# hediet/slideo

Hardware: AMD Instinct MI355X
Metric: frames/sec matched (1080p vs 500-page ORB set) (higher is better)
Workload: dtype u8

## Files before the change

### slideo_amd/csrc/orb.hip.h

```cpp
#pragma once
#include <limits.h>
#include <hip/hip_runtime.h>
#include <stdint.h>

#include "geom.h"
#include "types.h"
#include "cv_math.hip.h"

namespace slideo {

__global__ __launch_bounds__(256) void gray_kernel(const uint8_t* __restrict__ frames, int64_t frame_stride,
                                                   int stride, uint8_t* __restrict__ pyr, int64_t pyr_frame_bytes,
                                                   int w, int h, int pitch, int aligned4, GrayCoef gc) {
    const uint32_t half = 1u << (gc.shift - 1);
    auto gray_of = [&](uint32_t b, uint32_t g, uint32_t r) { return (__umul24(b, gc.cb) + __umul24(g, gc.cg) + __umul24(r, gc.cr) + half) >> gc.shift; };
    const int x = (blockIdx.x * 256 + threadIdx.x) * 4;
    const int y = blockIdx.y;
    if (x >= w) return;
    const uint8_t* src = frames + (int64_t)blockIdx.z * frame_stride + (int64_t)y * stride + (int64_t)x * 3;
    uint8_t* dst = pyr + (int64_t)blockIdx.z * pyr_frame_bytes + (int64_t)y * pitch + x;
    if (aligned4 && x + 3 < w) {
        const uint32_t* s = reinterpret_cast<const uint32_t*>(src);
        uint32_t a = s[0], b = s[1], c = s[2];
        uint32_t g0 = gray_of(a & 255, (a >> 8) & 255, (a >> 16) & 255);
        uint32_t g1 = gray_of(a >> 24, b & 255, (b >> 8) & 255);
        uint32_t g2 = gray_of((b >> 16) & 255, b >> 24, c & 255);
        uint32_t g3 = gray_of((c >> 8) & 255, (c >> 16) & 255, c >> 24);
        *reinterpret_cast<uint32_t*>(dst) = g0 | (g1 << 8) | (g2 << 16) | (g3 << 24);
    } else {
        for (int i = 0; i < 4 && x + i < w; ++i)
            dst[i] = (uint8_t)gray_of(src[3 * i], src[3 * i + 1], src[3 * i + 2]);
    }
}

__device__ __forceinline__ uint32_t dot2_u16(uint32_t a, uint32_t b, uint32_t c = 0u) {
    typedef unsigned short u16x2 __attribute__((ext_vector_type(2)));
    return __builtin_amdgcn_udot2(__builtin_bit_cast(u16x2, a), __builtin_bit_cast(u16x2, b), c, false);
}

constexpr int RESIZE_ROWS = 4;

__global__ __launch_bounds__(256) void resize_kernel(uint8_t* __restrict__ pyr, int64_t pyr_frame_bytes,
                                                     LevelGeom src, LevelGeom dst,
                                                     const uint32_t* __restrict__ lin_tab, int nxq, uint32_t nxq_magic) {
    const uint32_t t = blockIdx.x * 256 + threadIdx.x;
    const int yg = nxq_magic ? (int)__umulhi(t, nxq_magic) : (int)t;
    const int y0 = yg * RESIZE_ROWS;
    if (y0 >= dst.h) return;
    const int x0 = ((int)t - (int)__umul24(yg, nxq)) * 4;
    uint8_t* base = pyr + (int64_t)blockIdx.z * pyr_frame_bytes;
    const int nx = min(4, dst.w - x0);
    const uint4 xq = *reinterpret_cast<const uint4*>(lin_tab + dst.xtab_ofs + x0);
    const uint4 cq = *reinterpret_cast<const uint4*>(lin_tab + dst.xctab_ofs + x0);
    uint32_t ye[RESIZE_ROWS];
#pragma unroll
    for (int r = 0; r < RESIZE_ROWS; ++r) ye[r] = lin_tab[dst.ytab_ofs + min(y0 + r, dst.h - 1)];
    const uint32_t xe[4] = {xq.x, xq.y, xq.z, xq.w};
    const uint32_t cp[4] = {cq.x, cq.y, cq.z, cq.w};
    const int xs = min((int)(xe[0] & 0xffff), src.pitch - 8);
    const bool narrow = (int)(xe[3] & 0xffff) + 1 - xs < 8 || ((int)(xe[3] & 0xffff) - xs < 8 && (xe[3] >> 16) == 0);
    uint2 a[RESIZE_ROWS], b[RESIZE_ROWS];
#pragma unroll
    for (int r = 0; r < RESIZE_ROWS; ++r) {
        const int yo = ye[r] & 0xffff;
        const uint8_t* p0 = base + src.ofs + __umul24(yo, src.pitch) + xs;
        const uint8_t* p1 = base + src.ofs + __umul24(min(yo + 1, src.h - 1), src.pitch) + xs;
        __builtin_memcpy(&a[r], p0, 8);
        __builtin_memcpy(&b[r], p1, 8);
    }
#pragma unroll
    for (int r = 0; r < RESIZE_ROWS; ++r) {
        const int y = y0 + r;
        if (y >= dst.h) break;
        const int yo = ye[r] & 0xffff, cy1 = ye[r] >> 16, cy0 = 256 - cy1;
        uint32_t v[4];
        if (narrow) {
#pragma unroll
            for (int i = 0; i < 4; ++i) {
                const uint32_t pq = (uint32_t)((int)(xe[i] & 0xffff) - xs);
                const uint32_t sel = pq * 0x00010001u + 0x0c010c00u;
                const uint32_t ta = __builtin_amdgcn_perm(a[r].y, a[r].x, sel);
                const uint32_t tb = __builtin_amdgcn_perm(b[r].y, b[r].x, sel);
                v[i] = __umul24(cy0, dot2_u16(ta, cp[i])) + (__umul24(cy1, dot2_u16(tb, cp[i])) + (1u << 15));
            }
        } else {
            const uint8_t* r0 = base + src.ofs + __umul24(yo, src.pitch);
            const uint8_t* r1 = base + src.ofs + __umul24(min(yo + 1, src.h - 1), src.pitch);
#pragma unroll
            for (int i = 0; i < 4; ++i) {
                const int xo = xe[i] & 0xffff, cx1 = xe[i] >> 16, cx0 = 256 - cx1;
                const int xo1 = min(xo + 1, src.w - 1);
                uint32_t h0 = (uint32_t)cx0 * r0[xo] + (uint32_t)cx1 * r0[xo1];
                uint32_t h1 = (uint32_t)cx0 * r1[xo] + (uint32_t)cx1 * r1[xo1];
                v[i] = (uint32_t)cy0 * h0 + (uint32_t)cy1 * h1 + (1u << 15);
            }
        }
        const uint32_t outv = __builtin_amdgcn_perm(__builtin_amdgcn_perm(v[3], v[2], 0x0c0c0602u),
                                                    __builtin_amdgcn_perm(v[1], v[0], 0x0c0c0602u), 0x05040100u);
        uint8_t* d = base + dst.ofs + __umul24(y, dst.pitch) + x0;
        if (nx == 4) *reinterpret_cast<uint32_t*>(d) = outv;
        else for (int i = 0; i < nx; ++i) d[i] = (uint8_t)(outv >> (8 * i));
    }
}

__global__ __launch_bounds__(256) void resize_quad_kernel(uint8_t* __restrict__ pyr, int64_t pyr_frame_bytes,
                                                          LevelGeom src, LevelGeom dst,
                                                          const uint32_t* __restrict__ lin_tab, int nxq, uint32_t nxq_magic) {
    const uint32_t t = blockIdx.x * 256 + threadIdx.x;
    const uint32_t yg = nxq_magic ? __umulhi(t, nxq_magic) : t;
    const uint32_t y0 = yg * 4u;
    if ((int)y0 >= dst.h) return;
    const uint32_t q = t - __umul24(yg, (uint32_t)nxq);
    const uint8_t* __restrict__ sbase = pyr + (int64_t)blockIdx.z * pyr_frame_bytes + src.ofs;
    uint8_t* __restrict__ dbase = pyr + (int64_t)blockIdx.z * pyr_frame_bytes + dst.ofs;
    const uint4 sel4 = reinterpret_cast<const uint4*>(lin_tab + dst.xsel_ofs)[q];
    const uint4 cp4 = reinterpret_cast<const uint4*>(lin_tab + dst.xctab_ofs)[q];
    const uint32_t xs = lin_tab[dst.xs_ofs + q];
    const uint4 ye4 = *reinterpret_cast<const uint4*>(lin_tab + dst.ytab_ofs + y0);
    const uint32_t ye[4] = {ye4.x, ye4.y, ye4.z, ye4.w};
    const uint32_t sel[4] = {sel4.x, sel4.y, sel4.z, sel4.w}, cp[4] = {cp4.x, cp4.y, cp4.z, cp4.w};
    uint2 a[4], b[4];
#pragma unroll
    for (int r = 0; r < 4; ++r) {
        const uint32_t yo = ye[r] & 0xffffu;
        const uint32_t o0 = __umul24(yo, (uint32_t)src.pitch) + xs;
        const uint32_t o1 = __umul24(min(yo + 1u, (uint32_t)(src.h - 1)), (uint32_t)src.pitch) + xs;
        {
            const uint32_t sh = (xs & 3u) * 8u;
            uint32_t w0[3], w1[3];
            __builtin_memcpy(w0, sbase + (o0 & ~3u), 12);
            __builtin_memcpy(w1, sbase + (o1 & ~3u), 12);
            a[r] = make_uint2(__builtin_amdgcn_alignbit(w0[1], w0[0], sh), __builtin_amdgcn_alignbit(w0[2], w0[1], sh));
            b[r] = make_uint2(__builtin_amdgcn_alignbit(w1[1], w1[0], sh), __builtin_amdgcn_alignbit(w1[2], w1[1], sh));
        }
    }
    const uint32_t dofs = __umul24(y0, (uint32_t)dst.pitch) + 4u * q;
#pragma unroll
    for (int r = 0; r < 4; ++r) {
        const uint32_t cy1 = ye[r] >> 16, cy0 = 256u - cy1;
        uint32_t v[4];
#pragma unroll
        for (int i = 0; i < 4; ++i) {
            const uint32_t ta = __builtin_amdgcn_perm(a[r].y, a[r].x, sel[i]);
            const uint32_t tb = __builtin_amdgcn_perm(b[r].y, b[r].x, sel[i]);
            v[i] = __umul24(cy0, dot2_u16(ta, cp[i])) + (__umul24(cy1, dot2_u16(tb, cp[i])) + (1u << 15));
        }
        const uint32_t outv = __builtin_amdgcn_perm(__builtin_amdgcn_perm(v[3], v[2], 0x0c0c0602u),
                                                    __builtin_amdgcn_perm(v[1], v[0], 0x0c0c0602u), 0x05040100u);
        if ((int)(y0 + r) < dst.h) *reinterpret_cast<uint32_t*>(dbase + (dofs + (uint32_t)r * (uint32_t)dst.pitch)) = outv;
    }
}

__device__ __forceinline__ bool run9(uint32_t m) {
    m |= m << 16;
    m &= m >> 1; m &= m >> 2; m &= m >> 4; m &= m >> 1;
    return m != 0;
}

__device__ __forceinline__ int level_of_tile(const PyrGeom& g, int tile, bool blur) {
    int l = 0;
    for (int i = 1; i < g.nlevels; ++i) {
        int t0 = blur ? g.lv[i].btile0 : g.lv[i].ftile0;
        int n = blur ? g.lv[i].btx * g.lv[i].bty : g.lv[i].ftx * g.lv[i].fty;
        if (n > 0 && tile >= t0) l = i;
    }
    return l;
}

constexpr int FAST_SW = FAST_TW + 2, FAST_SH = FAST_TH + 2;
constexpr int FAST_XO = 4;
constexpr int FAST_RW = FAST_TW + 14, FAST_RH = FAST_TH + 8;
static_assert(FAST_SW == 128 && FAST_RW % 4 == 0 && (FAST_RW / 4) % 2 == 1 && FAST_RW >= FAST_SW + FAST_XO + 3, "fast_kernel maps one score row onto two wave-widths");

typedef short fast_s2 __attribute__((ext_vector_type(2)));
typedef unsigned short fast_us2 __attribute__((ext_vector_type(2)));
__device__ __forceinline__ fast_s2 fast_swap(fast_s2 a) { return __builtin_shufflevector(a, a, 1, 0); }

#ifndef FAST_TPB_V
#define FAST_TPB_V 8
#endif
constexpr int FAST_TPB = FAST_TPB_V;
constexpr int FAST_STAGE_CAP = 128;
constexpr int FAST_NDW = FAST_RW / 4;
constexpr int FAST_NLD = (FAST_RH + 6) / 7;

struct FastTile { int l, x0, y0; };

inline int4 fast_tile_entry(const PyrGeom& g, int tile_id) {
    int l = 0;
    for (int i = 1; i < g.nlevels; ++i) if (g.lv[i].ftx * g.lv[i].fty > 0 && tile_id >= g.lv[i].ftile0) l = i;
    const LevelGeom& L = g.lv[l];
    const int tile = tile_id - L.ftile0, ty = tile / (L.ftx > 0 ? L.ftx : 1), tx = tile - ty * L.ftx;
    const int x0 = L.rx0 + tx * FAST_TW, y0 = L.ry0 + ty * FAST_TH;
    return make_int4(l, x0, y0, 0);
}

__device__ __forceinline__ FastTile fast_tile_geo(const int4* __restrict__ tab, int tile_id) {
    const int4 e = tab[tile_id];
    FastTile T;
    T.l = e.x; T.x0 = e.y; T.y0 = e.z;
    return T;
}

__device__ __forceinline__ FastTile fast_tile_geo(const PyrGeom& g, int tile_id) {
    FastTile T;
    T.l = level_of_tile(g, tile_id, false);
    const LevelGeom& L = g.lv[T.l];
    const int tile = tile_id - L.ftile0;
    const int ty = tile / L.ftx, tx = tile - ty * L.ftx;
    T.x0 = L.rx0 + tx * FAST_TW; T.y0 = L.ry0 + ty * FAST_TH;
    return T;
}

constexpr int FAST_LT = 7 * FAST_NDW;
static_assert(FAST_LT <= 256 && 7 * FAST_NLD >= FAST_RH, "fast_kernel's loader covers the raw tile");

__device__ __forceinline__ void fast_issue_loads(const PyrGeom& g, const FastTile& T, const uint8_t* __restrict__ frame_pyr,
                                                 uint32_t (&v)[FAST_NLD], uint32_t& rel0, int& rel_level) {
    const LevelGeom& L = g.lv[T.l];
    const uint8_t* img = frame_pyr + L.ofs;
    const int xs = T.x0 - 1 - FAST_XO, maxo = L.pitch - 4;
    int tid = min((int)threadIdx.x, FAST_LT - 1);
    if (T.l != rel_level) {
        asm volatile("" : "+v"(tid));
        const int rg = tid / FAST_NDW, c = tid - rg * FAST_NDW;
        rel0 = __umul24((uint32_t)rg, (uint32_t)L.pitch) + 4u * (uint32_t)c;
        rel_level = T.l;
    }
    if (T.y0 >= 4 && T.y0 - 4 + 7 * FAST_NLD <= L.h && xs + FAST_RW <= L.pitch) {
        const uint32_t base = __umul24((uint32_t)(T.y0 - 4), (uint32_t)L.pitch) + (uint32_t)xs, step = 7u * (uint32_t)L.pitch;
#pragma unroll
        for (int k = 0; k < FAST_NLD; ++k) __builtin_memcpy(&v[k], img + (rel0 + (base + step * (uint32_t)k)), 4);
        return;
    }
    asm volatile("" : "+v"(tid));
    const int rg = tid / FAST_NDW, c = tid - rg * FAST_NDW;
#pragma unroll
    for (int k = 0; k < FAST_NLD; ++k) {
        const int gy = min(max(T.y0 - 4 + min(rg + 7 * k, FAST_RH - 1), 0), L.h - 1);
        __builtin_memcpy(&v[k], img + (__umul24((uint32_t)gy, (uint32_t)L.pitch) + (uint32_t)min(xs + 4 * c, maxo)), 4);
    }
}

__global__ __launch_bounds__(256) void fast_kernel(PyrGeom g, const uint8_t* __restrict__ pyr,
                                                   uint32_t* __restrict__ cand, uint32_t* __restrict__ cand_count,
                                                   uint32_t* __restrict__ hist, const int4* __restrict__ tile_tab) {
    __shared__ __attribute__((aligned(16))) uint8_t raw[FAST_RH][FAST_RW];
    __shared__ __attribute__((aligned(16))) uint8_t sc[FAST_SH][FAST_SW];
    constexpr int FAST_QR0 = (FAST_SH + 3) / 4, FAST_QR1 = (FAST_SH + 2) / 4, FAST_QR2 = (FAST_SH + 1) / 4;
    constexpr int FAST_PQ_TOTAL = 4 * 64 * (((FAST_SH * 32 + 255) / 256) + 3 * ((FAST_SH * 32 - 64 + 255) / 256));
    __shared__ uint16_t queue[FAST_PQ_TOTAL];
    __shared__ uint16_t gqueue[(FAST_QR0 + FAST_QR0 + FAST_QR0 + FAST_QR0) * 32];
    __shared__ uint32_t qcnt[4], gcnt[4];
    __shared__ uint32_t stage[FAST_STAGE_CAP], shist[256], nstage, stage_end, stage_base;
    const int f = blockIdx.y;
    const uint8_t* frame_pyr = pyr + (int64_t)f * g.frame_bytes;
    const int t = g.fast_thr;
    const int lane = threadIdx.x & 63, wave = __builtin_amdgcn_readfirstlane(threadIdx.x >> 6);
    const int first = blockIdx.x * FAST_TPB;
    FastTile T = fast_tile_geo(tile_tab, first);
    uint32_t pre[FAST_NLD], rel0 = 0;
    int rel_level = -1;
    fast_issue_loads(g, T, frame_pyr, pre, rel0, rel_level);
    shist[threadIdx.x] = 0;
    if (threadIdx.x == 0) { nstage = 0; stage_end = 0xFFFFFFFFu; }
    int stage_level = T.l;
    auto flush = [&](int lvl) {
        const uint32_t ns = min(min(nstage, (uint32_t)FAST_STAGE_CAP), stage_end);
        if (threadIdx.x == 0 && ns) stage_base = atomicAdd(cand_count + (size_t)f * g.nlevels + lvl, ns);
        __syncthreads();
        if (ns) {
            const LevelGeom& Ls = g.lv[lvl];
            uint32_t* clist = cand + (size_t)f * g.cand_per_frame + Ls.cand_ofs;
            const uint32_t base = stage_base;
            for (uint32_t i = threadIdx.x; i < ns; i += 256)
                if (base + i < (uint32_t)Ls.cand_cap) clist[base + i] = stage[i];
            const uint32_t hv = shist[threadIdx.x];
            if (hv) atomicAdd(hist + ((size_t)f * g.nlevels + lvl) * 256 + threadIdx.x, hv);
            shist[threadIdx.x] = 0;
        }
        __syncthreads();
        if (threadIdx.x == 0) { nstage = 0; stage_end = 0xFFFFFFFFu; }
    };
    for (int it = 0; it < FAST_TPB && first + it < g.fast_tiles; ++it) {
    if (it) {
        __syncthreads();
        if (T.l != stage_level || nstage > (uint32_t)FAST_STAGE_CAP / 2) flush(stage_level);
        stage_level = T.l;
    }
    if ((int)threadIdx.x < FAST_LT) {
#pragma unroll
        for (int k = 0; k < FAST_NLD; ++k) {
            const int i = (int)threadIdx.x + FAST_LT * k;
            if (i < FAST_NDW * FAST_RH) reinterpret_cast<uint32_t*>(&raw[0][0])[i] = pre[k];
        }
    }
    for (int i = threadIdx.x; i < FAST_SW * FAST_SH / 16; i += 256) reinterpret_cast<uint4*>(&sc[0][0])[i] = make_uint4(0, 0, 0, 0);
    const FastTile Tn = fast_tile_geo(tile_tab, min(first + it + 1, g.fast_tiles - 1));
    fast_issue_loads(g, Tn, frame_pyr, pre, rel0, rel_level);
    const int l = T.l;
    const LevelGeom& L = g.lv[l];
    const int x0 = T.x0, y0 = T.y0;
    constexpr int xoff = FAST_XO - 3;
    __syncthreads();
    const fast_us2 tt = {(unsigned short)t, (unsigned short)t};
    uint32_t myn = 0;
    constexpr int FAST_PQ0 = 4 * 64 * ((FAST_SH * 32 + 255) / 256), FAST_PQ1 = 4 * 64 * ((FAST_SH * 32 - 64 + 255) / 256),
                  FAST_PQ2 = 4 * 64 * ((FAST_SH * 32 - 128 + 255) / 256), FAST_PQ3 = 4 * 64 * ((FAST_SH * 32 - 192 + 255) / 256);
    static_assert(FAST_PQ0 + FAST_PQ1 + FAST_PQ2 + FAST_PQ3 <= FAST_PQ_TOTAL, "position queue");
    const int qbase = wave == 0 ? 0 : wave == 1 ? FAST_PQ0 : wave == 2 ? FAST_PQ0 + FAST_PQ1 : FAST_PQ0 + FAST_PQ1 + FAST_PQ2;
    uint16_t* const myq = queue + qbase;
    auto push1 = [&](bool cond, uint32_t val) {
        const uint64_t mk = __builtin_amdgcn_ballot_w64(cond);
        if (mk == 0ull) return;
        if (cond) myq[myn + __builtin_amdgcn_mbcnt_hi((uint32_t)(mk >> 32), __builtin_amdgcn_mbcnt_lo((uint32_t)mk, 0u))] = (uint16_t)val;
        myn += (uint32_t)__popcll(mk);
    };
    uint32_t myg = 0;
    uint16_t* const mygq = gqueue + (wave == 0 ? 0 : wave == 1 ? FAST_QR0 : wave == 2 ? FAST_QR0 + FAST_QR1 : FAST_QR0 + FAST_QR1 + FAST_QR2) * 32;
    const uint32_t* const rawdw = reinterpret_cast<const uint32_t*>(&raw[0][0]) + (FAST_XO >> 2);
    {
        const int half = lane >> 5, j = lane & 31;
        const bool colok = L.rx1 - (x0 - 1) - 4 * j + 1 > 0;
        for (int sy = wave; sy < FAST_SH; sy += 8) {
            if (y0 - 1 + sy > L.ry1) break;
            const int syl = min(sy + 4 * half, FAST_SH - 1);
            const bool rowok = sy + 4 * half < FAST_SH && y0 - 1 + syl <= L.ry1;
            const uint32_t* const c32 = rawdw + (syl + 3) * FAST_NDW + j;
            const uint32_t vc = c32[0], vt = c32[-3 * FAST_NDW], vb = c32[3 * FAST_NDW];
            const uint32_t sad = max(__builtin_amdgcn_sad_u8(vt, vc, 0u), __builtin_amdgcn_sad_u8(vb, vc, 0u));
            const bool flag = rowok && colok && sad > (uint32_t)t;
            const uint64_t mk = __builtin_amdgcn_ballot_w64(flag);
            if (mk == 0ull) continue;
            if (flag) mygq[myg + __builtin_amdgcn_mbcnt_hi((uint32_t)(mk >> 32), __builtin_amdgcn_mbcnt_lo((uint32_t)mk, 0u))] = (uint16_t)(syl * 32 + j);
            myg += (uint32_t)__popcll(mk);
        }
    }
    if (lane == 0) gcnt[wave] = myg;
    __syncthreads();
    const uint32_t gc1 = gcnt[0], gc2 = gc1 + gcnt[1], gc3 = gc2 + gcnt[2], ng = gc3 + gcnt[3];
    for (uint32_t k0 = 64u * (uint32_t)wave; k0 < ng; k0 += 256) {
        const uint32_t kq = min(k0 + lane, ng - 1u);
        const bool act = k0 + lane < ng;
        const uint32_t r = (kq >= gc1) + (kq >= gc2) + (kq >= gc3);
        const uint32_t e = gqueue[(r == 0 ? 0u : r == 1 ? (uint32_t)FAST_QR0 * 32 - gc1 : r == 2 ? (uint32_t)(FAST_QR0 + FAST_QR1) * 32 - gc2
                                                                                           : (uint32_t)(FAST_QR0 + FAST_QR1 + FAST_QR2) * 32 - gc3) + kq];
        const int syl = (int)(e >> 5), j = (int)(e & 31u);
        const uint32_t* const c32 = rawdw + (syl + 3) * FAST_NDW + j;
        const uint32_t c = c32[0], pv = c32[-1], nx = c32[1], vt = c32[-3 * FAST_NDW], vb = c32[3 * FAST_NDW];
        const uint32_t pc = c32[2 * FAST_NDW], pp = c32[2 * FAST_NDW - 1], pn = c32[2 * FAST_NDW + 1];
        const uint32_t mc = c32[-2 * FAST_NDW], mp = c32[-2 * FAST_NDW - 1], mn = c32[-2 * FAST_NDW + 1];
        auto pk = [](uint32_t hi, uint32_t lo, uint32_t sel) { return __builtin_bit_cast(fast_us2, __builtin_amdgcn_perm(hi, lo, sel)); };
        auto zero_or = [&](fast_us2 v, fast_us2 a, fast_us2 b, fast_us2 lo, fast_us2 hi) {
            return __builtin_elementwise_max(__builtin_elementwise_sub_sat(lo, __builtin_elementwise_min(a, b)),
                                             __builtin_elementwise_sub_sat(__builtin_elementwise_max(a, b), hi));
        };
        uint32_t keep[2];
#pragma unroll
        for (int par = 0; par < 2; ++par) {
            const uint32_t s0 = par ? 0x0c030c01u : 0x0c020c00u;
            const uint32_t s1 = par ? 0x0c040c02u : 0x0c030c01u;
            const uint32_t s2 = par ? 0x0c050c03u : 0x0c040c02u;
            const uint32_t s3 = par ? 0x0c060c04u : 0x0c050c03u;
            const fast_us2 v = pk(0u, c, s0);
            const fast_us2 lo = __builtin_elementwise_sub_sat(v, tt), hi = v + tt;
            fast_us2 d = zero_or(v, pk(0u, vt, s0), pk(0u, vb, s0), lo, hi);
            d = __builtin_elementwise_min(d, zero_or(v, pk(nx, c, s3), pk(c, pv, s1), lo, hi));
            d = __builtin_elementwise_min(d, zero_or(v, pk(pn, pc, s2), pk(mc, mp, s2), lo, hi));
            d = __builtin_elementwise_min(d, zero_or(v, pk(mn, mc, s2), pk(pc, pp, s2), lo, hi));
            keep[par] = __builtin_bit_cast(uint32_t, __builtin_elementwise_min(d, (fast_us2){1, 1}));
        }
        const uint32_t m = keep[0] | (keep[1] << 1);
        uint32_t fl = (m | (m >> 14)) & 0xFu;
        const int nin = min(max(L.rx1 - (x0 - 1) - 4 * j + 1, 0), 4);
        fl = act ? (fl & (nin >= 4 ? 0xFu : ((1u << nin) - 1u))) : 0u;
        if (__builtin_amdgcn_ballot_w64(fl != 0u) == 0ull) continue;
        const uint32_t p0 = (uint32_t)(syl * FAST_SW + 4 * j);
        push1((fl & 1u) != 0u, p0);
        push1((fl & 2u) != 0u, p0 + 1);
        push1((fl & 4u) != 0u, p0 + 2);
        push1((fl & 8u) != 0u, p0 + 3);
    }
    const uint32_t mym = myn;
    if (lane == 0) qcnt[wave] = mym;
    __syncthreads();
    const uint32_t qc1 = qcnt[0], qc2 = qc1 + qcnt[1], qc3 = qc2 + qcnt[2];
    auto qat = [&](uint32_t kq) -> int {
        const uint32_t r = (kq >= qc1) + (kq >= qc2) + (kq >= qc3);
        return queue[(r == 0 ? 0u : r == 1 ? (uint32_t)FAST_PQ0 - qc1 : r == 2 ? (uint32_t)(FAST_PQ0 + FAST_PQ1) - qc2
                                                                            : (uint32_t)(FAST_PQ0 + FAST_PQ1 + FAST_PQ2) - qc3) + kq];
    };
    const uint32_t nqueued = qc3 + qcnt[3];
    for (uint32_t kq = threadIdx.x; kq < nqueued; kq += 256) {
        const int i = qat(kq);
        const int sy = i >> 7, sx = i & 127;
        int score = 0;
        {
            const int cx = sx + 3 + xoff, cy = sy + 3;
            const int v = raw[cy][cx];
            int p[16];
            p[0] = raw[cy + 3][cx];     p[1] = raw[cy + 3][cx + 1]; p[2] = raw[cy + 2][cx + 2];
            p[3] = raw[cy + 1][cx + 3]; p[4] = raw[cy][cx + 3];     p[5] = raw[cy - 1][cx + 3];
            p[6] = raw[cy - 2][cx + 2]; p[7] = raw[cy - 3][cx + 1]; p[8] = raw[cy - 3][cx];
            p[9] = raw[cy - 3][cx - 1]; p[10] = raw[cy - 2][cx - 2]; p[11] = raw[cy - 1][cx - 3];
            p[12] = raw[cy][cx - 3];    p[13] = raw[cy + 1][cx - 3]; p[14] = raw[cy + 2][cx - 2];
            p[15] = raw[cy + 3][cx - 1];
            fast_s2 P[8];
#pragma unroll
            for (int k = 0; k < 8; ++k) P[k] = fast_s2{(short)(v - p[k]), (short)(v - p[k + 8])};
            fast_s2 n1[8], x1[8], n2[8], x2[8], n3[8], x3[8];
#pragma unroll
            for (int k = 0; k < 8; ++k) {
                const fast_s2 o = k < 7 ? P[k + 1] : fast_swap(P[0]);
                n1[k] = __builtin_elementwise_min(P[k], o); x1[k] = __builtin_elementwise_max(P[k], o);
            }
#pragma unroll
            for (int k = 0; k < 8; ++k) {
                const fast_s2 on = k < 6 ? n1[k + 2] : fast_swap(n1[k - 6]), ox = k < 6 ? x1[k + 2] : fast_swap(x1[k - 6]);
                n2[k] = __builtin_elementwise_min(n1[k], on); x2[k] = __builtin_elementwise_max(x1[k], ox);
            }
#pragma unroll
            for (int k = 0; k < 8; ++k) {
                const fast_s2 on = k < 4 ? n2[k + 4] : fast_swap(n2[k - 4]), ox = k < 4 ? x2[k + 4] : fast_swap(x2[k - 4]);
                n3[k] = __builtin_elementwise_min(n2[k], on); x3[k] = __builtin_elementwise_max(x2[k], ox);
            }
            fast_s2 bestv = {0, 0};
#pragma unroll
            for (int k = 0; k < 8; ++k) {
                const fast_s2 o = fast_swap(P[k]);
                const fast_s2 a9 = __builtin_elementwise_min(n3[k], o), b9 = __builtin_elementwise_max(x3[k], o);
                bestv = __builtin_elementwise_max(bestv, __builtin_elementwise_max(a9, (fast_s2){0, 0} - b9));
            }
            const int best = max((int)bestv.x, (int)bestv.y);
            score = best > t ? best - 1 : 0;
        }
        sc[sy][sx] = (uint8_t)score;
    }
    __syncthreads();
    uint32_t* ccount = cand_count + (size_t)f * g.nlevels + l;
    uint32_t* clist = cand + (size_t)f * g.cand_per_frame + L.cand_ofs;
    uint32_t* h = hist + ((size_t)f * g.nlevels + l) * 256;
    for (uint32_t k0 = 0; k0 < nqueued; k0 += 256) {
        const uint32_t kq = k0 + threadIdx.x;
        bool keep = false;
        int s = 0, gx = 0, gy = 0;
        if (kq < nqueued) {
            const int i = qat(kq);
            const int sy = i >> 7, sx = i & 127;
            gx = x0 - 1 + sx; gy = y0 - 1 + sy;
            if (sx >= 1 && sx <= FAST_TW && sy >= 1 && sy <= FAST_TH && gx < L.rx1 && gy < L.ry1) {
                const uint8_t* c = &sc[sy][sx];
                s = c[0];
                int m = max(max((int)c[-FAST_SW - 1], (int)c[-FAST_SW]), (int)c[-FAST_SW + 1]);
                m = max(max(m, (int)c[-1]), (int)c[1]);
                m = max(max(m, (int)c[FAST_SW - 1]), max((int)c[FAST_SW], (int)c[FAST_SW + 1]));
                keep = s > m;
            }
        }
        const uint64_t msk = __builtin_amdgcn_ballot_w64(keep);
        if (msk) {
            const uint32_t cnt = (uint32_t)__popcll(msk);
            uint32_t base = 0;
            if (lane == 0) base = atomicAdd(&nstage, cnt);
            base = __shfl(base, 0);
            const uint32_t entry = ((uint32_t)s << 24) | ((uint32_t)gy << 12) | (uint32_t)gx;
            if (base + cnt <= (uint32_t)FAST_STAGE_CAP) {
                if (keep) { stage[base + (uint32_t)__popcll(msk & ((1ull << lane) - 1ull))] = entry; atomicAdd(&shist[s], 1u); }
            } else {
                if (lane == 0) { atomicMin(&stage_end, base); base = atomicAdd(ccount, cnt); }
                base = __shfl(base, 0);
                if (keep) {
                    uint32_t pos = base + (uint32_t)__popcll(msk & ((1ull << lane) - 1ull));
                    if (pos < (uint32_t)L.cand_cap) clist[pos] = entry;
                    atomicAdd(h + s, 1u);
                }
            }
        }
    }
    T = Tn;
    }
    __syncthreads();
    flush(stage_level);
}

__device__ __forceinline__ int reflect101(int p, int n) {
    if (n == 1) return 0;
    while (p < 0 || p >= n) p = p < 0 ? -p : 2 * (n - 1) - p;
    return p;
}

typedef unsigned short blur_us2 __attribute__((ext_vector_type(2)));

__device__ __forceinline__ uint32_t blur_load_dword(const uint8_t* __restrict__ img, int pitch, int w, int gy, int xs) {
    const uint8_t* row = img + (int64_t)gy * pitch;
    if (xs >= 0 && xs + 3 < w) return *reinterpret_cast<const uint32_t*>(row + xs);
    uint32_t d = 0;
#pragma unroll
    for (int i = 0; i < 4; ++i) d |= (uint32_t)row[reflect101(xs + i, w)] << (8 * i);
    return d;
}

__global__ __launch_bounds__(256) void blur_kernel(PyrGeom g, const uint8_t* __restrict__ pyr,
                                                   uint8_t* __restrict__ blur, OrbTables const* __restrict__ tab) {
    const int f = blockIdx.y;
    const int l = level_of_tile(g, blockIdx.x, true);
    const LevelGeom L = g.lv[l];
    const int tile = blockIdx.x - L.btile0;
    const int ty = tile / L.btx, tx = tile - ty * L.btx;
    const int lane = threadIdx.x & 63, wave = threadIdx.x >> 6;
    const int x0 = tx * BLUR_TW;
    const int y0 = ty * BLUR_TH + wave * BLUR_RH;
    if (y0 >= L.h) return;
    const int xs = x0 - 4 + 4 * lane;
    const uint8_t* img = pyr + (int64_t)f * g.frame_bytes + L.ofs;
    uint8_t* out = blur + (int64_t)f * g.frame_bytes + L.ofs;
    uint32_t k[7];
#pragma unroll
    for (int i = 0; i < 7; ++i) k[i] = (uint32_t)tab->gk[i];
    uint32_t kk[7];
#pragma unroll
    for (int i = 0; i < 7; ++i) kk[i] = k[i] | (k[i] << 16);
    const uint32_t k01 = k[0] | (k[1] << 16), k12 = k[1] | (k[2] << 16), k23 = k[2] | (k[3] << 16), k34 = k[3] | (k[4] << 16),
                   k45 = k[4] | (k[5] << 16), k56 = k[5] | (k[6] << 16), k_0 = k[0] << 16, k6_ = k[6];
    uint32_t ra[7], rb[7];
    auto load = [&](int y) { return blur_load_dword(img, L.pitch, L.w, reflect101(y, L.h), xs); };
    auto unpack = [&](uint32_t d, uint32_t& A, uint32_t& B) {
        A = __builtin_amdgcn_perm(0u, d, 0x0C010C00u);
        B = __builtin_amdgcn_perm(0u, d, 0x0C030C02u);
    };
#pragma unroll
    for (int j = 0; j < 6; ++j) unpack(load(y0 - 3 + j), ra[j], rb[j]);
    const bool inner = lane >= 1 && lane <= 62;
    uint32_t dn0 = load(y0 + 3), dn1 = load(y0 + 4), dn2 = load(y0 + 5);
    for (int gI = 0; gI < BLUR_RH / 7; ++gI) {
#pragma unroll
        for (int ph = 0; ph < 7; ++ph) {
            const int i = gI * 7 + ph;
            unpack(dn0, ra[(ph + 6) % 7], rb[(ph + 6) % 7]);
            dn0 = dn1; dn1 = dn2;
            dn2 = load(min(y0 + i + 6, y0 + BLUR_RH + 2));
            uint32_t va = 0, vb = 0;
// ... 514 lines not shown
```

### slideo_amd/csrc/stage_orb.hip

```cpp
#include "runtime.hpp"
#include "orb.hip.h"
#include "yuv420.hip.h"
#include "reduce.hip.h"
#include "frame_mask.hip.h"

using namespace slideo;

namespace slideo {

static GrayCoef gray_coef(const slideo_matcher* m) {
    return m->cfg.ocv.gray == 1 ? GrayCoef{1868u, 9617u, 4899u, 14u} : GrayCoef{3735u, 19235u, 9798u, 15u};
}

void orb_stage_init(slideo_matcher* m) {
    const slideo_config* cfg = &m->cfg;
    OrbTables t{};
    umax_table(cfg->patch_size / 2, t.umax);
    if (cfg->ocv.blur == 2) gauss7_q8_rounded(t.gk); else gauss7_fixed(t.gk);
    gauss7_f32(t.gkf);
    brief_pattern(cfg->patch_size, t.pattern, cfg->ocv.rng_mul);
    m->d_tables.reserve(sizeof(OrbTables));
    HIP_CHECK(hipMemcpy(m->d_tables.p, &t, sizeof(t), hipMemcpyHostToDevice));
    std::vector<uint32_t> ict;
    ic_weight_table(cfg->patch_size / 2, t.umax, ict, m->ic_shift);
    m->ic_entries = (int)(ict.size() / 2);
    m->d_ictab.reserve(ict.size() * 4);
    HIP_CHECK(hipMemcpy(m->d_ictab.p, ict.data(), ict.size() * 4, hipMemcpyHostToDevice));
    HIP_CHECK(hipFuncSetAttribute(reinterpret_cast<const void*>(&describe_kernel), hipFuncAttributeMaxDynamicSharedMemorySize,
                                  describe_window(cfg->patch_size / 2).dwords * 16));
}

void orb_geom_init(slideo_matcher* m, GeomEntry& e, const std::vector<uint32_t>& lin_tab) {
    std::vector<uint32_t> tab = lin_tab;
    if (tab.empty()) tab.push_back(0);
    e.lin_tab.reserve(tab.size() * 4);
    HIP_CHECK(hipMemcpyAsync(e.lin_tab.p, tab.data(), tab.size() * 4, hipMemcpyHostToDevice, m->stream));
    std::vector<int4> ft((size_t)std::max(e.g.fast_tiles, 1));
    for (int t = 0; t < e.g.fast_tiles; ++t) ft[t] = fast_tile_entry(e.g, t);
    e.fast_tiles.reserve(ft.size() * sizeof(int4));
    HIP_CHECK(hipMemcpyAsync(e.fast_tiles.p, ft.data(), ft.size() * sizeof(int4), hipMemcpyHostToDevice, m->stream));
    HIP_CHECK(hipStreamSynchronize(m->stream));
}

void orb_launch_gray(const slideo_matcher* m, const uint8_t* frames_dev, int64_t frame_stride, int stride, uint8_t* gray, int64_t gframe, int w, int h,
                     int pitch, int n, hipStream_t st) {
    const int aligned4 = ((uintptr_t)frames_dev % 4 == 0) && (stride % 4 == 0) && (frame_stride % 4 == 0);
    gray_kernel<<<dim3(cdiv(cdiv(w, 4), 256), h, n), 256, 0, st>>>(frames_dev, frame_stride, stride, gray, gframe, w, h, pitch, aligned4, gray_coef(m));
    check_launch("gray_kernel");
}

void launch_yuv420_to_bgr(const uint8_t* src, int64_t src_fs, const slideo_yuv420_layout& L, int w, int h, int n, uint8_t* dst, hipStream_t st) {
    Yuv420Args a{};
    a.src = src; a.src_frame_stride = src_fs;
    a.interleaved = L.uv_step == 2;
    a.v_first = a.interleaved && L.v_offset < L.u_offset;
    a.c_ofs = a.interleaved ? std::min(L.u_offset, L.v_offset) : L.u_offset;
    a.v_ofs = L.v_offset;
    a.y_stride = L.y_stride; a.uv_stride = L.uv_stride;
    a.dst = dst; a.w = w; a.h = h;
    const bool luma4 = (uintptr_t)src % 4 == 0 && src_fs % 4 == 0 && L.y_stride % 4 == 0;
    const bool chroma = a.interleaved ? (a.c_ofs % 4 == 0 && L.uv_stride % 4 == 0)
                                      : (L.u_offset % 2 == 0 && L.v_offset % 2 == 0 && L.uv_stride % 2 == 0);
    const bool out4 = (uintptr_t)dst % 4 == 0 && w % 4 == 0;
    a.fast = luma4 && chroma && out4;
    dim3 grid(cdiv(cdiv(w, 4), YUV_TX), cdiv(h / 2, YUV_TY), n);
    yuv420_to_bgr_kernel<<<grid, dim3(YUV_TX, YUV_TY), 0, st>>>(a);
    check_launch("yuv420_to_bgr_kernel");
}

static ReduceEntry& reduce_for(slideo_matcher* m, int w, int h, int dw, int dh) {
    for (auto& r : m->reduces) if (r->ag.sw == w && r->ag.sh == h && r->ag.dw == dw && r->ag.dh == dh) return *r;
    auto e = std::make_unique<ReduceEntry>();
    std::vector<AreaTap> taps;
    std::vector<int32_t> idx;
    if (!build_area_geom_to(w, h, dw, dh, e->ag, taps, idx, m->cfg.ocv.area))
        fail(SLIDEO_ERR_INVALID_ARG, "reduce %dx%d -> %dx%d is not a shrink", w, h, dw, dh);
    e->d_taps.reserve(std::max<size_t>(taps.size() * sizeof(AreaTap), 16));
    e->d_idx.reserve(std::max<size_t>(idx.size() * 4, 16));
    HIP_CHECK(hipMemcpyAsync(e->d_taps.p, taps.data(), taps.size() * sizeof(AreaTap), hipMemcpyHostToDevice, m->stream));
    HIP_CHECK(hipMemcpyAsync(e->d_idx.p, idx.data(), idx.size() * 4, hipMemcpyHostToDevice, m->stream));
    HIP_CHECK(hipStreamSynchronize(m->stream));
    m->reduces.push_back(std::move(e));
    return *m->reduces.back();
}

void launch_reduce(slideo_matcher* m, const uint8_t* src, int64_t src_fs, int stride, int w, int h, int dw, int dh, int n, uint8_t* dst,
                   hipStream_t st) {
    const ReduceEntry& e = reduce_for(m, w, h, dw, dh);
    ReduceArgs a{};
    a.src = src; a.src_frame_stride = src_fs; a.src_stride = stride;
    a.dst = dst; a.sw = w; a.sh = h; a.dw = dw; a.dh = dh;
    a.ix = e.ag.iscale_x; a.iy = e.ag.iscale_y; a.inv_area = e.ag.fast_scale;
    a.out4 = (uintptr_t)dst % 4 == 0 && dw % 4 == 0;
    const dim3 grid(cdiv(cdiv(dw, 4), RED_TX), cdiv(dh, RED_TY), n), block(RED_TX, RED_TY);
    if (e.ag.fast) {
        const bool aligned = a.ix == 2 && a.iy == 2 && a.out4 && (uintptr_t)src % 8 == 0 && stride % 8 == 0 && src_fs % 8 == 0;
        if (aligned) reduce2x2_kernel<<<grid, block, 0, st>>>(a);
        else reduce_int_kernel<<<grid, block, 0, st>>>(a);
    } else {
        reduce_area_kernel<<<grid, block, 0, st>>>(a, e.ag, e.d_taps.as<AreaTap>(), e.d_idx.as<int32_t>());
    }
    check_launch("reduce kernel");
}

void orb_launch_scan(const uint32_t* counts, int n, uint32_t* qofs, uint32_t* info, hipStream_t st) {
    scan_kernel<<<1, 1024, 0, st>>>(counts, n, qofs, info);
    check_launch("scan_kernel");
}

static void launch_blur(slideo_matcher* m, Slot& S, const PyrGeom& g, int n, const uint8_t* strip_mask) {
    hipStream_t st = S.st;
    if (m->cfg.ocv.blur == 0)
        blur_f32_kernel<true><<<dim3(g.blur_tiles, n), 256, 0, st>>>(g, S.d_pyr.as<uint8_t>(), S.d_blur.as<uint8_t>(), m->d_tables.as<OrbTables>(), strip_mask);
    else if (m->cfg.ocv.blur == 1)
        blur_f32_kernel<false><<<dim3(g.blur_tiles, n), 256, 0, st>>>(g, S.d_pyr.as<uint8_t>(), S.d_blur.as<uint8_t>(), m->d_tables.as<OrbTables>(), strip_mask);
    else
        blur_kernel<<<dim3(g.blur_tiles, n), 256, 0, st>>>(g, S.d_pyr.as<uint8_t>(), S.d_blur.as<uint8_t>(), m->d_tables.as<OrbTables>());
    check_launch("blur kernel");
}

static bool resize_generic_forced() { return env_long("SLIDEO_RESIZE_GENERIC", 0) != 0; }

void orb_stage1(slideo_matcher* m, Slot& S, const DevFrames& f, int n, bool with_blur, uint32_t kp_cap, const uint8_t* mask_pyr) {
    hipStream_t st = S.st;
    const int w = f.w, h = f.h;
    const bool full_blur = with_blur;
    with_blur = with_blur || blur_is_f32(m);
    GeomEntry& ge = geom_for(m, w, h);
    const PyrGeom& g = ge.g;
    const int L = g.nlevels;
    S.d_pyr.reserve((size_t)g.frame_bytes * n + 256);
    if (with_blur) S.d_blur.reserve((size_t)g.frame_bytes * n);
    S.d_cand.reserve(std::max<size_t>((size_t)g.cand_per_frame * n * 4, 16));
    const size_t n_cc = (size_t)n * L;
    S.d_hist.reserve(n_cc * 256 * 4);
    S.d_candcount.reserve(n_cc * 2 * 4);
    S.d_flags.reserve(16);
    uint32_t* hist = S.d_hist.as<uint32_t>();
    uint32_t* cand_count = S.d_candcount.as<uint32_t>();
    uint32_t* flags = S.d_flags.as<uint32_t>();
    HIP_CHECK(hipMemsetAsync(hist, 0, n_cc * 256 * 4, st));
    HIP_CHECK(hipMemsetAsync(cand_count, 0, n_cc * 2 * 4, st));
    HIP_CHECK(hipMemsetAsync(flags, 0, 16, st));
    S.d_thr.reserve(n_cc * 4); S.d_lvlofs.reserve(n_cc * 4); S.d_kpcount.reserve((size_t)n * 4);
    S.d_qofs.reserve((size_t)(n + 1) * 4); S.d_info.reserve(64);
    S.h_info.reserve(64);

    const int aligned4 = ((uintptr_t)f.p % 4 == 0) && (f.stride % 4 == 0) && (f.frame_stride % 4 == 0);
    {
        dim3 grid(cdiv(cdiv(w, 4), 256), h, n);
        gray_kernel<<<grid, 256, 0, st>>>(f.p, f.frame_stride, f.stride, S.d_pyr.as<uint8_t>(), g.frame_bytes, w, h,
                                          g.lv[0].pitch, aligned4, gray_coef(m));
        check_launch("gray_kernel");
    }
    for (int l = 1; l < L; ++l) {
        if (g.lv[l].w <= 0 || g.lv[l].h <= 0) continue;
        const int nxq = cdiv(g.lv[l].w, 4);
        const uint32_t magic = nxq > 1 ? (uint32_t)(((1ull << 32) + (uint64_t)nxq - 1) / (uint64_t)nxq) : 0u;
        dim3 grid(cdiv(nxq * cdiv(g.lv[l].h, RESIZE_ROWS), 256), 1, n);
        if (g.lv[l].rq_ok && !resize_generic_forced())
            resize_quad_kernel<<<grid, 256, 0, st>>>(S.d_pyr.as<uint8_t>(), g.frame_bytes, g.lv[l - 1], g.lv[l], ge.lin_tab.as<uint32_t>(),
                                                     nxq, magic);
        else
            resize_kernel<<<grid, 256, 0, st>>>(S.d_pyr.as<uint8_t>(), g.frame_bytes, g.lv[l - 1], g.lv[l], ge.lin_tab.as<uint32_t>(),
                                                nxq, magic);
        check_launch("resize kernel");
    }
    if (g.fast_tiles > 0) {
        fast_kernel<<<dim3(cdiv(g.fast_tiles, FAST_TPB), n), 256, 0, st>>>(g, S.d_pyr.as<uint8_t>(), S.d_cand.as<uint32_t>(), cand_count, hist, ge.fast_tiles.as<int4>());
        check_launch("fast_kernel");
        if (mask_pyr) {
            mask_filter_kernel<<<dim3(L, n), MASK_BLOCK, 0, st>>>(g, mask_pyr, S.d_cand.as<uint32_t>(), cand_count, hist);
            check_launch("mask_filter_kernel");
        }
    }
    if (full_blur && g.blur_tiles > 0) launch_blur(m, S, g, n, nullptr);
    threshold_kernel<<<n, 64 * L, 0, st>>>(g, hist, cand_count, S.d_thr.as<uint32_t>(), S.d_lvlofs.as<uint32_t>(),
                                           S.d_kpcount.as<uint32_t>(), flags, kp_cap);
    check_launch("threshold_kernel");
    scan_kernel<<<1, 1024, 0, st>>>(S.d_kpcount.as<uint32_t>(), n, S.d_qofs.as<uint32_t>(), S.d_info.as<uint32_t>());
    check_launch("scan_kernel");
    HIP_CHECK(hipMemcpyAsync(S.h_info.p, S.d_info.p, 8, hipMemcpyDeviceToHost, st));
    HIP_CHECK(hipMemcpyAsync(S.h_info.as<uint32_t>() + 2, flags, 4, hipMemcpyDeviceToHost, st));
    S.orb.nframes = n;
    S.orb.full_blur = full_blur;
}

void orb_wait_info(slideo_matcher* m, Slot& S) {
    HIP_CHECK(hipStreamSynchronize(S.st));
    const uint32_t qtot = S.h_info.as<uint32_t>()[0], maxc = S.h_info.as<uint32_t>()[1], fl = S.h_info.as<uint32_t>()[2];
    if (fl & 1u) fail(SLIDEO_ERR_HIP, "internal: FAST candidate list overflow");
    S.orb.qtot = qtot; S.orb.max_count = maxc;
}

void orb_stage2(slideo_matcher* m, Slot& S, int w, int h, bool by_capacity) {
    hipStream_t st = S.st;
    const PyrGeom& g = geom_for(m, w, h).g;
    const int L = g.nlevels, n = S.orb.nframes;
    const uint32_t qtot = S.orb.qtot, maxc = S.orb.max_count;
    const uint32_t qtot_arg = by_capacity ? 0xFFFFFFFFu : qtot;
    S.d_items.reserve(std::max<size_t>((size_t)qtot * 8, 16));
    S.d_kp.reserve(std::max<size_t>((size_t)qtot * sizeof(slideo_keypoint), 16));
    S.d_desc.reserve(std::max<size_t>((size_t)qtot * 32, 32));
    if (qtot == 0) return;
    uint32_t* cand_count = S.d_candcount.as<uint32_t>();
    uint32_t* cursor = cand_count + (size_t)n * L;
    compact_kernel<<<dim3(L, n), 256, 0, st>>>(g, S.d_cand.as<uint32_t>(), cand_count, S.d_thr.as<uint32_t>(),
                                               S.d_lvlofs.as<uint32_t>(), S.d_qofs.as<uint32_t>(), cursor, S.d_items.as<uint64_t>());
    check_launch("compact_kernel");
    int np2 = 2;
    while ((uint32_t)np2 < maxc && np2 < KP_SORT_LDS) np2 <<= 1;
    sort_kernel<<<n, 1024, (size_t)np2 * 8, st>>>(S.d_qofs.as<uint32_t>(), S.d_items.as<uint64_t>(), np2);
    check_launch("sort_kernel");
    if (maxc > (uint32_t)np2) {
        sort_global_kernel<<<n, 1024, 0, st>>>(S.d_qofs.as<uint32_t>(), S.d_items.as<uint64_t>(), (uint32_t)np2);
        check_launch("sort_global_kernel");
    }
    if (blur_is_f32(m)) {
        if (!S.orb.full_blur && g.blur_tiles > 0) {
            const size_t mask_bytes = (size_t)n * g.blur_tiles * 4;
            S.d_blurmask.reserve(mask_bytes);
            HIP_CHECK(hipMemsetAsync(S.d_blurmask.p, 0, mask_bytes, st));
            blur_mark_kernel<<<cdiv((int)qtot, 256), 256, 0, st>>>(g, S.d_qofs.as<uint32_t>(), n, S.d_items.as<uint64_t>(), qtot_arg, S.d_blurmask.as<uint8_t>());
            check_launch("blur_mark_kernel");
            launch_blur(m, S, g, n, S.d_blurmask.as<uint8_t>());
        }
        describe_blurred_kernel<<<cdiv((int)qtot, 4), 256, 0, st>>>(g, S.d_pyr.as<uint8_t>(), S.d_blur.as<uint8_t>(), m->d_tables.as<OrbTables>(),
                                                                    S.d_qofs.as<uint32_t>(), n, S.d_items.as<uint64_t>(), qtot_arg,
                                                                    m->d_ictab.as<uint2>(), m->ic_shift, m->ic_entries,
                                                                    S.d_kp.as<slideo_keypoint>(), S.d_desc.as<uint8_t>(), m->cfg.ocv.atan);
        check_launch("describe_blurred_kernel");
        return;
    }
    const DescWin dw = describe_window(g.half_patch);
    describe_kernel<<<cdiv((int)qtot, 4), 256, (size_t)dw.dwords * 16, st>>>(g, S.d_pyr.as<uint8_t>(), m->d_tables.as<OrbTables>(),
                                                                             S.d_qofs.as<uint32_t>(), n, S.d_items.as<uint64_t>(), qtot_arg, dw,
                                                                             m->d_ictab.as<uint2>(), m->ic_shift, m->ic_entries,
// ... 50 lines not shown
```

Before: 24230.

## Vectorize gray conversion with udot4 and 16-pixel loads; branchless FAST queue indexing

Rewrites the BGR-to-gray kernel so each thread handles 16 pixels with 128-bit loads and stores and computes weights via packed udot4 dot products, using a flattened 1D grid with magic-number division. Also replaces the FAST kernel's nested ternary queue-offset lookup with a select-based helper and makes the NMS and row-flag loops branchless by clamping indices. The aim is fewer memory transactions and less ALU/divergence per pixel. Rounding of the gray value is changed to a 16-bit fixed-point rescale of the coefficients, which could differ slightly from the original if the shift exceeds 16.

Measured after the change: 24180. Within noise of the previous version (-0.2%).

```diff
diff --git a/slideo_amd/csrc/orb.hip.h b/slideo_amd/csrc/orb.hip.h
--- a/slideo_amd/csrc/orb.hip.h
+++ b/slideo_amd/csrc/orb.hip.h
@@ -9,27 +9,51 @@
 
 namespace slideo {
 
+struct GrayDot { uint32_t lo4, hi4; };
+
+inline GrayDot gray_dot(GrayCoef gc) {
+    const uint32_t s = 16u - gc.shift, b = gc.cb << s, g = gc.cg << s, r = gc.cr << s;
+    return GrayDot{(b & 255u) | (g & 255u) << 8 | (r & 255u) << 16, (b >> 8) | (g >> 8) << 8 | (r >> 8) << 16};
+}
+
+__device__ __forceinline__ uint32_t gray_sum(uint32_t p, GrayDot gd) {
+    return (__builtin_amdgcn_udot4(p, gd.hi4, 0u, false) << 8) + __builtin_amdgcn_udot4(p, gd.lo4, 1u << 15, false);
+}
+
+__device__ __forceinline__ uint32_t gray_quad(uint32_t a, uint32_t b, uint32_t c, GrayDot gd) {
+    const uint32_t s0 = gray_sum(a, gd), s1 = gray_sum(__builtin_amdgcn_alignbit(b, a, 24), gd);
+    const uint32_t s2 = gray_sum(__builtin_amdgcn_alignbit(c, b, 16), gd), s3 = gray_sum(c >> 8, gd);
+    return __builtin_amdgcn_perm(s1, s0, 0x0c0c0602u) | __builtin_amdgcn_perm(s3, s2, 0x06020c0cu);
+}
+
+constexpr int GRAY_PX = 16;
+
+template <int PX>
 __global__ __launch_bounds__(256) void gray_kernel(const uint8_t* __restrict__ frames, int64_t frame_stride,
                                                    int stride, uint8_t* __restrict__ pyr, int64_t pyr_frame_bytes,
-                                                   int w, int h, int pitch, int aligned4, GrayCoef gc) {
-    const uint32_t half = 1u << (gc.shift - 1);
-    auto gray_of = [&](uint32_t b, uint32_t g, uint32_t r) { return (__umul24(b, gc.cb) + __umul24(g, gc.cg) + __umul24(r, gc.cr) + half) >> gc.shift; };
-    const int x = (blockIdx.x * 256 + threadIdx.x) * 4;
-    const int y = blockIdx.y;
-    if (x >= w) return;
-    const uint8_t* src = frames + (int64_t)blockIdx.z * frame_stride + (int64_t)y * stride + (int64_t)x * 3;
+                                                   int w, int h, int pitch, int aligned4, GrayDot gd,
+                                                   int ngx, uint32_t ngx_magic) {
+    const uint32_t t = blockIdx.x * 256 + threadIdx.x;
+    const int y = ngx_magic ? (int)__umulhi(t, ngx_magic) : (int)t;
+    if (y >= h) return;
+    const int x = ((int)t - (int)__umul24(y, ngx)) * PX;
+    const uint8_t* src = frames + (int64_t)blockIdx.z * frame_stride + (int64_t)y * stride + x * 3;
     uint8_t* dst = pyr + (int64_t)blockIdx.z * pyr_frame_bytes + (int64_t)y * pitch + x;
-    if (aligned4 && x + 3 < w) {
-        const uint32_t* s = reinterpret_cast<const uint32_t*>(src);
-        uint32_t a = s[0], b = s[1], c = s[2];
-        uint32_t g0 = gray_of(a & 255, (a >> 8) & 255, (a >> 16) & 255);
-        uint32_t g1 = gray_of(a >> 24, b & 255, (b >> 8) & 255);
-        uint32_t g2 = gray_of((b >> 16) & 255, b >> 24, c & 255);
-        uint32_t g3 = gray_of((c >> 8) & 255, (c >> 16) & 255, c >> 24);
-        *reinterpret_cast<uint32_t*>(dst) = g0 | (g1 << 8) | (g2 << 16) | (g3 << 24);
-    } else {
-        for (int i = 0; i < 4 && x + i < w; ++i)
-            dst[i] = (uint8_t)gray_of(src[3 * i], src[3 * i + 1], src[3 * i + 2]);
+    if (PX == GRAY_PX && x + GRAY_PX <= w) {
+        const uint4* s = reinterpret_cast<const uint4*>(src);
+        const uint4 u = s[0], v = s[1], q = s[2];
+        *reinterpret_cast<uint4*>(dst) = make_uint4(gray_quad(u.x, u.y, u.z, gd), gray_quad(u.w, v.x, v.y, gd),
+                                                    gray_quad(v.z, v.w, q.x, gd), gray_quad(q.y, q.z, q.w, gd));
+        return;
+    }
+    for (int i = 0; i < PX && x + i < w; i += 4) {
+        if (aligned4 && x + i + 3 < w) {
+            const uint32_t* s = reinterpret_cast<const uint32_t*>(src + 3 * i);
+            *reinterpret_cast<uint32_t*>(dst + i) = gray_quad(s[0], s[1], s[2], gd);
+        } else {
+            for (int k = i; k < i + 4 && x + k < w; ++k)
+                dst[k] = (uint8_t)(gray_sum(src[3 * k] | (uint32_t)src[3 * k + 1] << 8 | (uint32_t)src[3 * k + 2] << 16, gd) >> 16);
+        }
     }
 }
 
@@ -185,6 +209,14 @@
 constexpr int FAST_NLD = (FAST_RH + 6) / 7;
 
 struct FastTile { int l, x0, y0; };
+
+__device__ __forceinline__ uint32_t fast_quarter_index(uint32_t k, uint32_t c1, uint32_t c2, uint32_t c3, uint32_t b1, uint32_t b2, uint32_t b3) {
+    uint32_t o = 0u;
+    o = k >= c1 ? b1 - c1 : o;
+    o = k >= c2 ? b2 - c2 : o;
+    o = k >= c3 ? b3 - c3 : o;
+    return o + k;
+}
 
 inline int4 fast_tile_entry(const PyrGeom& g, int tile_id) {
     int l = 0;
@@ -322,14 +354,14 @@
     {
         const int half = lane >> 5, j = lane & 31;
         const bool colok = L.rx1 - (x0 - 1) - 4 * j + 1 > 0;
-        for (int sy = wave; sy < FAST_SH; sy += 8) {
-            if (y0 - 1 + sy > L.ry1) break;
-            const int syl = min(sy + 4 * half, FAST_SH - 1);
-            const bool rowok = sy + 4 * half < FAST_SH && y0 - 1 + syl <= L.ry1;
+        const int nrow = min(FAST_SH, L.ry1 - (y0 - 1) + 1);
+        const int mylim = colok ? nrow : 0;
+        for (int sy = wave; sy < nrow; sy += 8) {
+            const int syu = sy + 4 * half, syl = min(syu, FAST_SH - 1);
             const uint32_t* const c32 = rawdw + (syl + 3) * FAST_NDW + j;
             const uint32_t vc = c32[0], vt = c32[-3 * FAST_NDW], vb = c32[3 * FAST_NDW];
             const uint32_t sad = max(__builtin_amdgcn_sad_u8(vt, vc, 0u), __builtin_amdgcn_sad_u8(vb, vc, 0u));
-            const bool flag = rowok && colok && sad > (uint32_t)t;
+            const bool flag = (syu < mylim) & (sad > (uint32_t)t);
             const uint64_t mk = __builtin_amdgcn_ballot_w64(flag);
             if (mk == 0ull) continue;
             if (flag) mygq[myg + __builtin_amdgcn_mbcnt_hi((uint32_t)(mk >> 32), __builtin_amdgcn_mbcnt_lo((uint32_t)mk, 0u))] = (uint16_t)(syl * 32 + j);
@@ -342,9 +374,7 @@
     for (uint32_t k0 = 64u * (uint32_t)wave; k0 < ng; k0 += 256) {
         const uint32_t kq = min(k0 + lane, ng - 1u);
         const bool act = k0 + lane < ng;
-        const uint32_t r = (kq >= gc1) + (kq >= gc2) + (kq >= gc3);
-        const uint32_t e = gqueue[(r == 0 ? 0u : r == 1 ? (uint32_t)FAST_QR0 * 32 - gc1 : r == 2 ? (uint32_t)(FAST_QR0 + FAST_QR1) * 32 - gc2
-                                                                                           : (uint32_t)(FAST_QR0 + FAST_QR1 + FAST_QR2) * 32 - gc3) + kq];
+        const uint32_t e = gqueue[fast_quarter_index(kq, gc1, gc2, gc3, FAST_QR0 * 32, (FAST_QR0 + FAST_QR1) * 32, (FAST_QR0 + FAST_QR1 + FAST_QR2) * 32)];
         const int syl = (int)(e >> 5), j = (int)(e & 31u);
         const uint32_t* const c32 = rawdw + (syl + 3) * FAST_NDW + j;
         const uint32_t c = c32[0], pv = c32[-1], nx = c32[1], vt = c32[-3 * FAST_NDW], vb = c32[3 * FAST_NDW];
@@ -386,9 +416,7 @@
     __syncthreads();
     const uint32_t qc1 = qcnt[0], qc2 = qc1 + qcnt[1], qc3 = qc2 + qcnt[2];
     auto qat = [&](uint32_t kq) -> int {
-        const uint32_t r = (kq >= qc1) + (kq >= qc2) + (kq >= qc3);
-        return queue[(r == 0 ? 0u : r == 1 ? (uint32_t)FAST_PQ0 - qc1 : r == 2 ? (uint32_t)(FAST_PQ0 + FAST_PQ1) - qc2
-                                                                            : (uint32_t)(FAST_PQ0 + FAST_PQ1 + FAST_PQ2) - qc3) + kq];
+        return queue[fast_quarter_index(kq, qc1, qc2, qc3, FAST_PQ0, FAST_PQ0 + FAST_PQ1, FAST_PQ0 + FAST_PQ1 + FAST_PQ2)];
     };
     const uint32_t nqueued = qc3 + qcnt[3];
     for (uint32_t kq = threadIdx.x; kq < nqueued; kq += 256) {
@@ -440,23 +468,19 @@
     uint32_t* ccount = cand_count + (size_t)f * g.nlevels + l;
     uint32_t* clist = cand + (size_t)f * g.cand_per_frame + L.cand_ofs;
     uint32_t* h = hist + ((size_t)f * g.nlevels + l) * 256;
+    const int rx1 = L.rx1, ry1 = L.ry1;
     for (uint32_t k0 = 0; k0 < nqueued; k0 += 256) {
         const uint32_t kq = k0 + threadIdx.x;
-        bool keep = false;
-        int s = 0, gx = 0, gy = 0;
-        if (kq < nqueued) {
-            const int i = qat(kq);
-            const int sy = i >> 7, sx = i & 127;
-            gx = x0 - 1 + sx; gy = y0 - 1 + sy;
-            if (sx >= 1 && sx <= FAST_TW && sy >= 1 && sy <= FAST_TH && gx < L.rx1 && gy < L.ry1) {
-                const uint8_t* c = &sc[sy][sx];
-                s = c[0];
-                int m = max(max((int)c[-FAST_SW - 1], (int)c[-FAST_SW]), (int)c[-FAST_SW + 1]);
-                m = max(max(m, (int)c[-1]), (int)c[1]);
-                m = max(max(m, (int)c[FAST_SW - 1]), max((int)c[FAST_SW], (int)c[FAST_SW + 1]));
-                keep = s > m;
-            }
-        }
+        const int i = qat(min(kq, nqueued - 1u));
+        const int sy = i >> 7, sx = i & 127;
+        const int gx = x0 - 1 + sx, gy = y0 - 1 + sy;
+        const bool inside = (kq < nqueued) & (sx >= 1) & (sx <= FAST_TW) & (sy >= 1) & (sy <= FAST_TH) & (gx < rx1) & (gy < ry1);
+        const uint8_t* c = &sc[min(max(sy, 1), FAST_TH)][min(max(sx, 1), FAST_TW)];
+        const int s = c[0];
+        int m = max(max((int)c[-FAST_SW - 1], (int)c[-FAST_SW]), (int)c[-FAST_SW + 1]);
+        m = max(max(m, (int)c[-1]), (int)c[1]);
+        m = max(max(m, (int)c[FAST_SW - 1]), max((int)c[FAST_SW], (int)c[FAST_SW + 1]));
+        const bool keep = inside & (s > m);
         const uint64_t msk = __builtin_amdgcn_ballot_w64(keep);
         if (msk) {
             const uint32_t cnt = (uint32_t)__popcll(msk);
diff --git a/slideo_amd/csrc/stage_orb.hip b/slideo_amd/csrc/stage_orb.hip
--- a/slideo_amd/csrc/stage_orb.hip
+++ b/slideo_amd/csrc/stage_orb.hip
@@ -44,8 +44,16 @@
 
 void orb_launch_gray(const slideo_matcher* m, const uint8_t* frames_dev, int64_t frame_stride, int stride, uint8_t* gray, int64_t gframe, int w, int h,
                      int pitch, int n, hipStream_t st) {
-    const int aligned4 = ((uintptr_t)frames_dev % 4 == 0) && (stride % 4 == 0) && (frame_stride % 4 == 0);
-    gray_kernel<<<dim3(cdiv(cdiv(w, 4), 256), h, n), 256, 0, st>>>(frames_dev, frame_stride, stride, gray, gframe, w, h, pitch, aligned4, gray_coef(m));
+    auto aligned = [&](uintptr_t a) {
+        return ((uintptr_t)frames_dev % a == 0) && (stride % a == 0) && (frame_stride % a == 0) && ((uintptr_t)gray % a == 0) && (pitch % a == 0) && (gframe % a == 0);
+    };
+    const int px = aligned(16) ? GRAY_PX : 4, ngx = cdiv(w, px);
+    const uint32_t magic = ngx > 1 ? (uint32_t)(((1ull << 32) + (uint64_t)ngx - 1) / (uint64_t)ngx) : 0u;
+    const dim3 grid(cdiv(ngx * h, 256), 1, n);
+    if (px == GRAY_PX)
+        gray_kernel<GRAY_PX><<<grid, 256, 0, st>>>(frames_dev, frame_stride, stride, gray, gframe, w, h, pitch, 1, gray_dot(gray_coef(m)), ngx, magic);
+    else
+        gray_kernel<4><<<grid, 256, 0, st>>>(frames_dev, frame_stride, stride, gray, gframe, w, h, pitch, aligned(4), gray_dot(gray_coef(m)), ngx, magic);
     check_launch("gray_kernel");
 }
 
@@ -146,13 +154,7 @@
     S.d_qofs.reserve((size_t)(n + 1) * 4); S.d_info.reserve(64);
     S.h_info.reserve(64);
 
-    const int aligned4 = ((uintptr_t)f.p % 4 == 0) && (f.stride % 4 == 0) && (f.frame_stride % 4 == 0);
-    {
-        dim3 grid(cdiv(cdiv(w, 4), 256), h, n);
-        gray_kernel<<<grid, 256, 0, st>>>(f.p, f.frame_stride, f.stride, S.d_pyr.as<uint8_t>(), g.frame_bytes, w, h,
-                                          g.lv[0].pitch, aligned4, gray_coef(m));
-        check_launch("gray_kernel");
-    }
+    orb_launch_gray(m, f.p, f.frame_stride, f.stride, S.d_pyr.as<uint8_t>(), g.frame_bytes, w, h, g.lv[0].pitch, n, st);
     for (int l = 1; l < L; ++l) {
         if (g.lv[l].w <= 0 || g.lv[l].h <= 0) continue;
         const int nxq = cdiv(g.lv[l].w, 4);
```
